# TUMFTM/CamRaDepth

Measured on AMD Instinct MI355X. Metric: training images/sec at 256x416 bf16, higher is better.
Workload: dtype bf16; 1 GPU; CamRaDepth base (image+radar) train step, 8x7x256x416 per GPU, bf16 MFMA / fp32 accumulate, diffGradNorm + OneCycleLR, Dropout2d/DropPath on; global_batch=8, parallelism=dp1, hip_graph=True

## Files before the change

camradepth_amd/csrc/wgrad3x3.hip:

```cpp
#include <stdlib.h>
#include "common.h"

namespace {

struct Wg3K {
  const bf16_t* x; int x_ld; int Cin;
  const bf16_t* dy; int dy_ld; int Cout;
  int B, H, W;
  int strips_x;
  int rows_per_wg;
  int S, nchunks;
  long long total_rows;
  long long x_bytes, dy_bytes;
  crd_sum_t* dw; crd_sum_t* dbias;
  float* dw_part;
};

constexpr int XS = 6, YS = 4;
constexpr int XPX = 40;
constexpr int XLD = 64;
typedef __attribute__((address_space(3))) void* lds_ptr;
template <int N>
__device__ __forceinline__ void wait_vm() { asm volatile("s_waitcnt vmcnt(%0)" ::"n"(N) : "memory"); }

__device__ __forceinline__ int swz128(int r) { return (r & 3) ^ ((r >> 3) & 1); }
__device__ __forceinline__ int swz256(int r) { return (r & 3) | (((r >> 3) & 1) << 2); }
__device__ __forceinline__ int swz192(int r) { return (r >> 3) & 1; }
template <int COT>
__device__ __forceinline__ int swz_y(int r) { return COT == 128 ? swz256(r) : (COT == 96 ? swz192(r) : (COT == 64 ? swz128(r) : 0)); }

__device__ __forceinline__ s16x4 tr_read3(const bf16_t* p) {
  return __builtin_amdgcn_ds_read_tr16_b64_v4i16((__attribute__((address_space(3))) s16x4*)(p));
}

template <int WCO, int WCI, int TCO, int RPS>
__global__ __launch_bounds__(512) void k_wgrad3x3(Wg3K a) {
  constexpr int XSr = XS * RPS, YSr = YS * RPS;
  static_assert(WCO * WCI == 8, "8 waves");
  constexpr int NT = 4 / WCI;
  constexpr int COT = WCO * TCO * 16;
  constexpr int YGRP = 32 * COT * 2 / 1024;
  extern __shared__ __attribute__((aligned(16))) bf16_t lds[];
  bf16_t* sX = lds;
  bf16_t* sY = lds + XSr * XPX * XLD;

  const int t = threadIdx.x, l = t & 63;
  const int wv = __builtin_amdgcn_readfirstlane(t >> 6);
  const int wco = wv / WCI, wci = wv % WCI;
  const int chunk = (int)blockIdx.x / a.S, split = (int)blockIdx.x - chunk * a.S;
  const int c0 = chunk * XLD;
  const unsigned OOB = 0x80000000u;

  f32x4 acc[9][TCO][NT];
#pragma unroll
  for (int tp = 0; tp < 9; ++tp)
#pragma unroll
    for (int i = 0; i < TCO; ++i)
#pragma unroll
      for (int j = 0; j < NT; ++j) acc[tp][i][j] = f32x4{0.f, 0.f, 0.f, 0.f};
  const int q = l >> 4, prow = (l & 15) >> 2, pcol = (l & 3) * 4;
  int yoff[TCO][2], xoff[3][NT][2];
#pragma unroll
  for (int i = 0; i < TCO; ++i)
#pragma unroll
    for (int h = 0; h < 2; ++h) {
      const int r = 8 * q + prow + 4 * h;
      yoff[i][h] = r * COT + (((wco * TCO + i) ^ swz_y<COT>(r)) << 4) + pcol;
    }
#pragma unroll
  for (int kx = 0; kx < 3; ++kx)
#pragma unroll
    for (int j = 0; j < NT; ++j)
#pragma unroll
      for (int h = 0; h < 2; ++h) {
        const int r = 8 * q + prow + kx + 4 * h;
        xoff[kx][j][h] = r * XLD + (((wci * NT + j) ^ swz128(r)) << 4) + pcol;
      }
  const bool do_bias = a.dbias != nullptr && chunk == 0 && t < a.Cout;
  float bsum = 0.f;

  long long sr = (long long)split * a.rows_per_wg;
  long long sr_end = sr + a.rows_per_wg;
  if (sr_end > a.total_rows) sr_end = a.total_rows;

  const int xpix = 8 * wv + (l >> 3);
  const int xgr = l & 7;
  const int ylin = 64 * wv + l;
  const int ypix = ylin / (COT / 8);
  const int ygr = ylin % (COT / 8);

  while (sr < sr_end) {
    const long long strip = sr / a.H;
    const int y0 = (int)(sr - strip * a.H);
    long long seg_end = (strip + 1) * a.H;
    if (seg_end > sr_end) seg_end = sr_end;
    const int y1 = y0 + (int)(seg_end - sr);
    const int b = __builtin_amdgcn_readfirstlane((int)(strip / a.strips_x));
    const int sx = (int)(strip - (long long)b * a.strips_x);
    const int x0 = sx * 32;
    const crd_rsrc_t rx = make_rsrc(a.x + (long long)b * a.H * a.W * a.x_ld, (unsigned)a.x_bytes);
    const crd_rsrc_t ry = make_rsrc(a.dy + (long long)b * a.H * a.W * a.dy_ld, (unsigned)a.dy_bytes);

    auto issue_x = [&](int h) {
#if defined(__HIP_DEVICE_COMPILE__)
      if (wv < 5) {
        const int ix = x0 - 1 + xpix, ch = c0 + ((((xgr >> 1) ^ swz128(xpix)) << 1) | (xgr & 1)) * 8;
        const bool ok = (unsigned)h < (unsigned)a.H && (unsigned)ix < (unsigned)a.W && xpix < 34 && ch < a.Cin;
        const unsigned off = ok ? (unsigned)((((long long)h * a.W + ix) * a.x_ld + ch) * 2) : OOB;
        lds_dma16(rx, (unsigned)(uintptr_t)(lds_ptr)(sX + (((h + 1) % XSr) * XPX + 8 * wv) * XLD), off);
      }
#else
      (void)h;
#endif
    };
    auto issue_y = [&](int r) {
#if defined(__HIP_DEVICE_COMPILE__)
      if (wv < YGRP) {
        const int ix = x0 + ypix, co = ((((ygr >> 1) ^ swz_y<COT>(ypix)) << 1) | (ygr & 1)) * 8;
        const bool ok = r < y1 && ix < a.W && co < a.Cout;
        const unsigned off = ok ? (unsigned)((((long long)r * a.W + ix) * a.dy_ld + co) * 2) : OOB;
        lds_dma16(ry, (unsigned)(uintptr_t)(lds_ptr)(sY + (r % YSr) * 32 * COT + 512 * wv), off);
      }
#else
      (void)r;
#endif
    };

    asm volatile("s_waitcnt vmcnt(0) lgkmcnt(0)\n\ts_barrier" ::: "memory");
    issue_x(y0 - 1);
    issue_x(y0);
#pragma unroll
    for (int s = 0; s < 3; ++s)
#pragma unroll
      for (int r = 0; r < RPS; ++r) { issue_y(y0 + s * RPS + r); issue_x(y0 + s * RPS + 1 + r); }

    for (int y = y0; y < y1; y += RPS) {
      if (wv < 5 && wv < YGRP) wait_vm<4 * RPS>();
      else if (wv < 5 || wv < YGRP) wait_vm<2 * RPS>();
      asm volatile("s_waitcnt lgkmcnt(0)\n\ts_barrier" ::: "memory");
#pragma unroll
      for (int r = 0; r < RPS; ++r) { issue_y(y + 3 * RPS + r); issue_x(y + 3 * RPS + 1 + r); }

      const bool mfma_on = c0 + wci * NT * 16 < a.Cin;
      if (!mfma_on && !do_bias) continue;
#pragma unroll
      for (int rr = 0; rr < RPS; ++rr) {
        const int yy = y + rr;
        if (rr > 0 && yy >= y1) break;
        const bf16_t* yrow = sY + (yy % YSr) * 32 * COT;
        if (mfma_on) {
        bf16x8 af[TCO];
#pragma unroll
        for (int i = 0; i < TCO; ++i) {
          s16x4 lo = tr_read3(yrow + yoff[i][0]), hi = tr_read3(yrow + yoff[i][1]);
          union { bf16x8 v; s16x4 h[2]; } u;
          u.h[0] = lo; u.h[1] = hi;
          af[i] = u.v;
        }
#pragma unroll
        for (int ky = 0; ky < 3; ++ky) {
          const bf16_t* xrow = sX + ((yy + ky) % XSr) * XPX * XLD;
#pragma unroll
          for (int kx = 0; kx < 3; ++kx) {
#pragma unroll
            for (int j = 0; j < NT; ++j) {
              s16x4 lo = tr_read3(xrow + xoff[kx][j][0]), hi = tr_read3(xrow + xoff[kx][j][1]);
              union { bf16x8 v; s16x4 h[2]; } u;
              u.h[0] = lo; u.h[1] = hi;
#pragma unroll
              for (int i = 0; i < TCO; ++i)
                acc[ky * 3 + kx][i][j] = __builtin_amdgcn_mfma_f32_16x16x32_bf16(af[i], u.v, acc[ky * 3 + kx][i][j], 0, 0, 0);
            }
          }
        }
        }
        if (do_bias) {
#pragma unroll 8
          for (int r = 0; r < 32; ++r) bsum += bf2f(yrow[r * COT + ((((t >> 4) ^ swz_y<COT>(r)) << 4) | (t & 15))]);
        }
      }
    }
    sr = seg_end;
  }

  const int Ktot = 9 * a.Cin;
#pragma unroll
  for (int tp = 0; tp < 9; ++tp)
#pragma unroll
    for (int i = 0; i < TCO; ++i)
#pragma unroll
      for (int j = 0; j < NT; ++j) {
        const int ci = c0 + (wci * NT + j) * 16 + (l & 15);
#pragma unroll
        for (int r = 0; r < 4; ++r) {
          const int co = (wco * TCO + i) * 16 + (l >> 4) * 4 + r;
          if (co < a.Cout && ci < a.Cin) {
            const long long off = (long long)co * Ktot + tp * a.Cin + ci;
            if (a.dw_part) a.dw_part[(long long)split * a.Cout * Ktot + off] = acc[tp][i][j][r];
            else grad_add(a.dw + off, acc[tp][i][j][r]);
          }
        }
      }
  if (do_bias) grad_add(a.dbias + t, bsum);
}

int plan_rows(long long total_rows, int Cin, int& rows_per_wg, int budget, int cap) {
  const int chunks = cdiv(Cin, XLD);
  const int W = budget > 0 ? budget : 256;
  long long S = W / chunks;
  if (S < 1) S = 1;
  if (cap > 0 && S > cap) S = cap;
  if (S > total_rows / 8) S = total_rows / 8 > 0 ? total_rows / 8 : 1;
  rows_per_wg = (int)((total_rows + S - 1) / S);
  return (int)((total_rows + rows_per_wg - 1) / rows_per_wg);
}

template <int WCO, int WCI, int TCO, int RPS>
int launch_w3r(const Wg3K& k0, hipStream_t st, int budget, int partial_capacity) {
  Wg3K k = k0;
  constexpr int COT = WCO * TCO * 16;
  const size_t lds = (size_t)RPS * (XS * XPX * XLD + YS * 32 * COT) * sizeof(bf16_t);
  k.nchunks = cdiv(k.Cin, XLD);
  k.S = plan_rows(k.total_rows, k.Cin, k.rows_per_wg, budget, k.dw_part ? partial_capacity : 0);
  static bool attr_done = false;
  if (!attr_done) {
    crd_reserve_lds(reinterpret_cast<const void*>(&k_wgrad3x3<WCO, WCI, TCO, RPS>), (int)lds, "k_wgrad3x3");
    attr_done = true;
  }
  hipLaunchKernelGGL((k_wgrad3x3<WCO, WCI, TCO, RPS>), dim3(k.nchunks * k.S), dim3(512), lds, st, k);
  CRD_LAUNCH_CHECK("crd_conv_wgrad(3x3 streaming)");
  return CRD_OK;
}

template <int WCO, int WCI, int TCO>
int launch_w3(const Wg3K& k, hipStream_t st, int budget, int partial_capacity) {
  static int rps = -1;
  if (rps < 0) rps = crd_dev_int("CRD_W3_RPS", 2);
  return rps == 1 ? launch_w3r<WCO, WCI, TCO, 1>(k, st, budget, partial_capacity) : launch_w3r<WCO, WCI, TCO, 2>(k, st, budget, partial_capacity);
}

}

int crd_wgrad3x3_stream(const crd_wgrad_desc* d, hipStream_t st) {
  Wg3K k;
  k.x = reinterpret_cast<const bf16_t*>(d->x) + d->x_coff; k.x_ld = d->x_ld; k.Cin = d->Cin;
  k.dy = reinterpret_cast<const bf16_t*>(d->dy) + d->dy_coff; k.dy_ld = d->dy_ld; k.Cout = d->Cout;
  k.B = d->B; k.H = d->IH; k.W = d->IW;
  k.strips_x = cdiv(d->IW, 32);
  k.total_rows = (long long)d->B * k.strips_x * d->IH;
  k.rows_per_wg = 0;
  k.x_bytes = (long long)d->IH * d->IW * d->x_ld * 2;
  k.dy_bytes = (long long)d->IH * d->IW * d->dy_ld * 2;
  CRD_UNSUPPORTED(k.x_bytes < (1ll << 31) && k.dy_bytes < (1ll << 31), "crd_conv_wgrad: image too large for 32-bit byte offsets");
  k.dw = d->dw; k.dbias = d->dbias;
  k.dw_part = d->dw_partials;
  CRD_CHECK_ARG(d->dw_partials == nullptr || d->dw_partial_capacity >= 1, "crd_conv_wgrad: dw_partials needs a capacity >= 1");
  CRD_CHECK_ARG(d->wg_budget >= 0, "crd_conv_wgrad: wg_budget must be >= 0");
  if (d->Cout <= 32) return launch_w3<2, 4, 1>(k, st, d->wg_budget, d->dw_partial_capacity);
  if (d->Cout <= 64) return launch_w3<2, 4, 2>(k, st, d->wg_budget, d->dw_partial_capacity);
  if (d->Cout <= 96) return launch_w3<2, 4, 3>(k, st, d->wg_budget, d->dw_partial_capacity);
  if (crd_dev_int("CRD_W3_T22", 0)) return launch_w3<4, 2, 2>(k, st, d->wg_budget, d->dw_partial_capacity);
  return launch_w3<2, 4, 4>(k, st, d->wg_budget, d->dw_partial_capacity);
}

int crd_wgrad3x3_splits(const crd_wgrad_desc* d) {
  int rows = 0;
  return plan_rows((long long)d->B * cdiv(d->IW, 32) * d->IH, d->Cin, rows, d->wg_budget, d->dw_partial_capacity > 0 ? d->dw_partial_capacity : 0);
}
```

camradepth_amd/engine.py:

```python
import bisect
import ctypes as C
import os

import torch

from . import lib as L
from . import trace
from .config import MID_CHANNELS, UNSUP_CLASSES, ModelConfig
from .params import short_res_block_plan

_DEV = os.environ.get("CRD_DEV_SWITCHES") == "1"


def _dev_flag(name):
    return _DEV and os.environ.get(name) is not None


def _dev_int(name, default):
    return int(os.environ.get(name, default)) if _DEV else int(default)


GROUP_WGRAD = not _dev_flag("CRD_NO_GROUP_WGRAD")
SIDE_STREAMS = _dev_flag("CRD_SIDE_STREAMS")
FUSE_GN_RED = _dev_flag("CRD_FUSE_GN_RED")
# ... 74 lines not shown
        return "k_igemm<2,2,1,1>"
    if cout <= 32:
        return "k_igemm<4,1,1,1>"
    if cout <= 64:
        return "k_igemm<2,2,2,1>"
    if cout <= 96:
        return "k_igemm<4,1,1,3>"
    if 128 < cout <= 160:
        return "k_igemm<4,1,1,5>"
    return "k_igemm<2,2,2,2>"


KCAT = _dev_int("CRD_KCAT", 1) != 0
GNB_FC1 = _dev_int("CRD_GNB_FC1", 7)
GNB_SR = _dev_int("CRD_GNB_SR", 15)
QSR_GROUP = _dev_int("CRD_QSR_GROUP", 4)
FUSE_NORM2_APPLY = not _dev_flag("CRD_NO_FUSE_NORM2_APPLY")
FUSE_BLOCK_RED = not _dev_flag("CRD_NO_FUSE_BLOCK_RED")


def fused_reduce_tile_ok(cout, ohw, B):
    small = cout > 32 and -(-ohw // 128) * -(-cout // 128) * B < 192
    return FUSE_BLOCK_RED and cout % 16 == 0 and (small or cout <= 64 or 96 < cout <= 128 or cout > 160)


def persistent_conv3(spec, B):
    if os.environ.get("CRD_CONV3P", "1") == "0":
        return False
    y = spec["y"]
    plain = (not y.f32 and spec["bias"] is None and not spec["act"] and spec["res"] is None and spec["out_mode"] == 0
             and spec.get("red") is None and spec.get("chan") is None)
    halo = spec["k"] == 3 and spec["stride"] == 1 and spec["OW"] >= 32 and spec["OH"] >= 8
    tiles = -(-spec["OW"] // 32) * -(-spec["OH"] // 16) * B
    return bool(plain and halo and tiles >= 192 and spec["cout"] >= 64 and spec["cout"] % 8 == 0)


def halo_tile(cout, OH=1 << 20, OW=1 << 20, B=1):
    tiles = -(-OW // 32) * -(-OH // 8) * B
    if cout > 32 and tiles * -(-cout // 128) < 512:
        return "k_conv3x3<4,1,2,2>" if tiles * -(-cout // 64) >= 512 else "k_conv3x3<4,1,2,1>"
    if cout <= 32:
        return "k_conv3x3<4,1,2,1>"
    if cout <= 64:
        return "k_conv3x3<4,1,2,2>"
    if cout <= 96:
        return "k_conv3x3<4,1,2,3>"
    if 128 < cout <= 160 or 256 < cout <= 320:
        return "k_conv3x3<4,1,2,4>+<4,1,2,1>" if cout - (256 if cout > 256 else 128) <= 32 else "k_conv3x3<4,1,2,4>+<4,1,2,2>"
    return "k_conv3x3<4,1,2,4>"


def wgrad_tile(cout):
    if cout <= 32:
        return "k_wgrad<1,4,2,2>"
    if cout <= 64:
        return "k_wgrad<1,4,4,2>"
    if cout <= 96:
        return "k_wgrad<2,2,3,4>"
    return "k_wgrad<2,2,4,4>"


class ConvW:

    def __init__(self, name, cout, cin_ref, k, cmap, bias, need_dgrad, scatter=False, dgrad_rows=None):
        self.name, self.cout, self.cin_ref, self.k, self.taps = name, cout, cin_ref, k, k * k
        self.cmap = cmap
        self.cin_pad = len(cmap) if cmap is not None else rup(cin_ref)
        self.cout_pad = rup(cout)
        self.bias, self.need_dgrad, self.scatter = bias, need_dgrad, scatter
        self.identity = (cmap is None and self.cin_pad == cin_ref and self.taps == 1)
        self.w_fwd = self.w_dgrad = self.w_scatter = None
        self.dw = None
        self.wg_budget = 0
        self.dw_parts, self.dw_S, self.stream3_geom = None, 0, None
        self.cmap_dev = None


class Plan:
    def __init__(self, model, B, H, W, training):
        cfg = model.cfg
        assert H % 32 == 0 and W % 32 == 0, "H and W must be multiples of 32 (SURVEY.md section 8 note on 900x1600)"
        self.model, self.cfg, self.B, self.H, self.W, self.training = model, cfg, B, H, W, training
        self.dev = model.flat.device
        self.lib = L.load()
        self.fwd, self.bwd_groups, self.bwd_tags = [], [], []
        self._tag = "enc0"
        self.zero_fwd, self.zero_bwd = [], []
        self._zf_views, self._zb_views = [], []
        self.convs = []
        self.keep = []
        self.dw_entries, self.dw_grads = [], []
        self.row_grads = []
        self.kcat_entries = []
        self.shapes = {}
        self.fwd_marks = []
        self._defer = None
        self._cur_stream = 0
        self._side_streams = None
        self.split_late = False
        self.attn_parts = None
        self.mlp_parts = None
        self.stats_scratch = None
        self.buffers = []
        self.gn_conv_on = gn_conv_default()
        self.enc_taps = {}
        self.block_ops = {}
        self.need_grad = bool(getattr(model, "_need_grad", True))
        self.frozen = frozenset(n for n in model._names if not model._param(n).requires_grad)
        self._dump = {}
        f8 = getattr(model, "fp8_scales", None)
        self.fp8_keep_bf16 = bool(training or self.need_grad)
        self.fp8 = dict(f8) if (f8 and (not self.fp8_keep_bf16 or getattr(model, "fp8_train", False))) else None
        self.fp8_convs = []
        self.fp8_kcat = []
        self.fp8_grad = bool(self.fp8 is not None and training and getattr(model, "fp8_grad", False))
        self.fp8_grad_layers, self.fp8_jit, self.fp8_margin = [], True, 2.0
        if self.fp8_grad:
            self.g8_scales = torch.ones(16, dtype=F32, device=self.dev)
            self.g8_amax = torch.zeros((16, 64), dtype=torch.int32, device=self.dev)
            self.buffers += [self.g8_scales, self.g8_amax]
        self._build()

    def new(self, shape, dtype=BF16):
        t = torch.zeros(shape, dtype=dtype, device=self.dev)
        self.buffers.append(t)
        if os.environ.get("CRD_DEBUG_NAN"):
            import traceback
            fr = [f"{f.name}:{f.lineno}" for f in traceback.extract_stack()[-5:-1]]
            self.keep.append(("buf", len(self.keep), tuple(shape), str(dtype), fr, t))
        return t

    def act(self, C_, H, W, dtype=BF16, ld=None):
        return PM(self.new((self.B, H * W, ld or C_), dtype), C_, H, W)

    def zf(self, *shape):
        v = _Lazy(shape)
        self._zf_views.append(v)
        return v

    def zb(self, *shape):
        v = _Lazy(shape)
        self._zb_views.append(v)
        return v

    def _materialise(self, views):
        n = sum(v.numel for v in views)
        arena = torch.zeros(max(n, 1), dtype=SUM, device=self.dev)
        off = 0
        for v in views:
            v.t = arena[off:off + v.numel].view(v.shape)
            off += v.numel
        return arena

    def _emit(self, lst, fn_name, args, region=None, acc_slot=None, io=None):
        op = Op(getattr(self.lib, fn_name), list(args), fn_name, region, acc_slot, stream=self._cur_stream, io=io)
        lst.append(op)
        return op

    def live(self, op):
        return op.fn is not None and (op.cond is None or getattr(self, op.cond[0]) == op.cond[1])

    @staticmethod
    def op_bytes(op):
        io = op.io
        return int(io() if callable(io) else (io or 0))

    class _Side:
        def __init__(self, plan, s):
            self.plan, self.s = plan, s

        def __enter__(self):
            self.prev, self.plan._cur_stream = self.plan._cur_stream, self.s

        def __exit__(self, *a):
            self.plan._cur_stream = self.prev

    def side(self, s):
        return Plan._Side(self, s if SIDE_STREAMS else 0)

    def join(self, lst, s):
        if SIDE_STREAMS:
            lst.append(Op(None, [], "join", stream=s))

    def _push(self, grp):
        self.bwd_groups.append(grp)
        self.bwd_tags.append(self._tag)

    def conv_desc(self, x, w_t, cout, k, stride, pad, OH, OW, y, cin=None, gather=0, out_mode=0, patch_k=0, patch_c=0,
                  bias=None, bias_bstride=0, act=0, res=None, res_scale=None, stats=None, accumulate=0, red=None, chan=None):
        return dict(x=x, w=w_t, cout=cout, k=k, stride=stride, pad=pad, OH=OH, OW=OW, y=y, cin=cin if cin is not None else x.C,
                    gather=gather, out_mode=out_mode, patch_k=patch_k, patch_c=patch_c, bias=bias, bias_bstride=bias_bstride,
                    act=act, res=res, res_scale=res_scale, stats=stats, accumulate=accumulate, red=red, chan=chan)

    def conv(self, lst, spec, region=None):
        w, x = spec["w"], spec["x"]
        if isinstance(w, tuple) and w[0] == "kcat":
            flops = spec["flops_override"]
        elif isinstance(w, tuple):
            cw = w[1]
            flops = 2.0 * self.B * x.H * x.W * cw.cout * cw.taps * min(spec["cout"] // (cw.taps if w[0] == "scatter" else 1),
                                                                         cw.cin_ref)
        else:
            flops = 2.0 * self.B * spec["OH"] * spec["OW"] * spec["cout"] * w.cin_ref * w.taps
        halo = spec["k"] == 3 and spec["stride"] == 1 and spec["out_mode"] == 0 and spec["OW"] >= 32 and spec["OH"] >= 8
        cout = spec["cout"]
        covered = cout <= 160 or 256 < cout <= 320
        if (halo and SPLIT_N and cout > 128 and 0 < cout % 128 <= 64 and not covered and spec["bias"] is None
                and spec["stats"] is None and spec["res"] is None and "w_row0" not in spec):
            c_main = cout // 128 * 128
            for c0, c1 in ((0, c_main), (c_main, cout)):
                sub = dict(spec)
                sub.update(cout=c1 - c0, y=spec["y"].sl(c0, c1), w_row0=c0, flops_override=flops * (c1 - c0) / cout)
                self.conv(lst, sub, None if region is None else region[:-2] + (region[-2] + c0, region[-2] + c1))
            return None
        flops = spec.get("flops_override", flops)
        kname = halo_tile(spec["cout"], spec["OH"], spec["OW"], self.B) if halo else igemm_tile(spec["cout"], spec["OH"] * spec["OW"], self.B)
        if self._narrow_takes(spec, False):
            kname = "k_pw_narrow"
        if halo and persistent_conv3(spec, self.B):
            c = spec["cout"]
            rest = c % 128
            kname = "k_conv3x3p<2>" if c <= 64 else "k_conv3x3p<3>" if c <= 96 else "k_conv3x3p<4>" + ("" if rest == 0 or rest > 64 else
                                                                                                 "+k_conv3x3<4,1,2,1>" if rest <= 32 else "+k_conv3x3<4,1,2,2>")
        meta = {"kernel": kname, "flops": flops,
                "shape": f"{('dgrad-kcat' if w[0] == 'kcat' else 'dgrad') if isinstance(w, tuple) else 'fwd'} Cin{spec['cin']} Cout{spec['cout']} k{spec['k']} s{spec['stride']} "
                         f"out{spec['OH']}x{spec['OW']}"}
        wbytes = spec["cout"] * spec["k"] * spec["k"] * spec["cin"] * 2

        def io(spec=spec, wbytes=wbytes):
            xs, ys = spec["x"], spec["y"]
            n = xs.t.shape[0] * xs.P * spec["cin"] * (4 if xs.f32 else 2) + wbytes
            n += nbytes(ys) * (2 if spec["accumulate"] else 1) + nbytes(spec["res"])
            if spec.get("red") is not None:
                n += nbytes(spec["red"][0])
            return n
        op = Op(self.lib.crd_conv_igemm, [spec], "crd_conv_igemm", region, ("spec", spec) if region else None, meta,
                stream=self._cur_stream, io=io)
        lst.append(op)
        return op

    def _narrow_takes(self, spec, with_gn):
        y = spec["y"]
        if not (spec["k"] == 1 and spec["stride"] == 1 and spec["out_mode"] == 0 and not spec["act"] and not spec["accumulate"]
                and (with_gn or spec["cin"] == 512)
                and int(self.lib.crd_pw_narrow_supported(spec["cin"], spec["cout"], spec["OH"] * spec["OW"])) > 0):
            return False
        if y.f32:
            return spec.get("red") is None
        red = spec.get("red")
        return spec["res"] is None and spec["stats"] is None and spec.get("chan") is None and (red is None or red[5] == 0)

    def gn_conv(self, lst, spec, stats, gmul, gname, act, xn):
        w, x = spec["w"], spec["x"]
        assert x.coff == 0 and (xn is None or xn.coff == 0)
        flops = 2.0 * self.B * spec["OH"] * spec["OW"] * spec["cout"] * w.cin_ref * w.taps
        small = spec["cout"] <= 64 or -(-spec["OH"] * spec["OW"] // 64) * -(-spec["cout"] // 128) * self.B < 256
        kname = "k_gngemm_reg" + ("<2,2,1,1>" if small else "<2,2,1,2>")
        if act and not x.f32 and self._narrow_takes(spec, True):
            kname = "k_pw_narrow<gn+gelu>"
        meta = {"kernel": kname, "flops": flops,
                "shape": f"gn+fwd Cin{spec['cin']} Cout{spec['cout']} k{spec['k']} s{spec['stride']} out{spec['OH']}x{spec['OW']}"}
        gn = dict(gn_in=True, x_f32=x.f32, gmul=gmul, stats=stats, gamma=self.p(gname + ".weight"), beta=self.p(gname + ".bias"),
                  act=act, xn=xn)
        io = nbytes(x, spec["y"], xn, spec["res"]) + spec["cout"] * spec["cin"] * 2
        op = Op(self.lib.crd_gn_conv, [spec, gn], "crd_gn_conv", None, None, meta, stream=self._cur_stream, io=io)
        lst.append(op)
        return op

    def gn_bwd_conv(self, lst, spec, gx, stats, gmul, gname, act, r, dx, mask=None):
        w, x = spec["w"], spec["x"]
        cw = w[1]
        assert isinstance(w, tuple) and x.coff == 0 and gx.coff == 0 and (dx is None or dx.coff == 0) and spec["k"] == 1
        flops = 2.0 * self.B * x.H * x.W * cw.cout * cw.taps * min(spec["cout"] // (cw.taps if w[0] == "scatter" else 1), cw.cin_ref)
        small = spec["cout"] <= 64 or -(-spec["OH"] * spec["OW"] // 64) * -(-spec["cout"] // 128) * self.B < 256 or spec["out_mode"] == 1
        kname = "k_gnbwd_gemm" + ("<1>" if small else "<2>")
        meta = {"kernel": kname, "flops": flops,
                "shape": f"gnbwd+{'scatter' if w[0] == 'scatter' else 'dgrad'} Cin{spec['cin']} Cout{spec['cout']} out{spec['OH']}x{spec['OW']}"}
        frozen = self.is_frozen(gname + ".weight", gname + ".bias")
        gnb = dict(gnb_in=True, gx=gx, gmul=gmul, act=act, stats=stats, gamma=self.p(gname + ".weight"), beta=self.p(gname + ".bias"),
                   mask=mask, r=r, dx=dx, dgamma=None if frozen else self.g(gname + ".weight"), dbeta=None if frozen else self.g(gname + ".bias"))

        def io(spec=spec, x=x, gx=gx, dx=dx):
            n = nbytes(x, gx, dx) + spec["cout"] * spec["cin"] * 2
            n += nbytes(spec["y"]) * (2 if spec["accumulate"] else 1)
            if spec.get("red") is not None:
                n += nbytes(spec["red"][0])
            return n
        op = Op(self.lib.crd_gn_bwd_conv, [spec, gnb], "crd_gn_bwd_conv", None, None, meta, stream=self._cur_stream, io=io)
        lst.append(op)
        return op

    def wgrad(self, lst, x, dy, cw, k, stride, pad, OH, OW, dbias=None, cin=None):
        if cw.frozen:
            return
        if dbias is not None:
            rows = self.zb(cw.cout)
            self.row_grads.append((dbias, cw.cout, rows, 1, cw.tag, 0, cw.cout))
            dbias = rows
        spec = dict(wg=True, x=x, dy=dy, cw=cw, k=k, stride=stride, pad=pad, OH=OH, OW=OW, dbias=dbias,
                    cin=cin if cin is not None else x.C)
        stream3 = k == 3 and stride == 1 and OW >= 32 and OH >= 8
        if stream3:
            cw.stream3_geom = (x.H, x.W, spec["cin"])
        kname = ("k_wgrad3x3<2,4,1>" if cw.cout <= 32 else "k_wgrad3x3<2,4,2>" if cw.cout <= 64 else "k_wgrad3x3<2,4,3>" if cw.cout <= 96 else "k_wgrad3x3<2,4,4>") if stream3 \
            else wgrad_tile(cw.cout)
        meta = {"kernel": kname, "flops": 2.0 * self.B * OH * OW * cw.cout * cw.cin_ref * cw.taps, "param": cw.name,
                "shape": f"wgrad Cin{spec['cin']} Cout{cw.cout} k{k} s{stride} out{OH}x{OW}"}
        meta["bytes"] = x.t.shape[0] * x.P * spec["cin"] * (4 if x.f32 else 2) + nbytes(dy) + cw.cout * cw.taps * spec["cin"] * 4
        if self._defer is not None and not stream3:
            self._defer.append((spec, meta))
            return
        stream = LATE if self._cur_stream == 0 else self._cur_stream
        lst.append(Op(self.lib.crd_conv_wgrad, [spec], "crd_conv_wgrad", meta=meta, stream=stream, io=meta["bytes"]))

    def flush_deferred(self, lst):
        items, self._defer = self._defer, None
        if not items:
            return
        meta = {"kernel": "k_wgrad_grouped", "flops": sum(m["flops"] for _, m in items), "shape": f"{len(items)} wgrads",
                "params": [m["param"] for _, m in items]}
        lst.append(Op(self.lib.crd_conv_wgrad_grouped, [{"wg_group": [sp for sp, _ in items]}], "crd_conv_wgrad_grouped", meta=meta,
                      stream=LATE, io=sum(m["bytes"] for _, m in items)))

    def _make_group(self, specs):
        descs = (L.WgradDesc * len(specs))()
        for i, sp in enumerate(specs):
            self._make_desc(sp, into=descs[i])
        info = L.WgradGroupInfo()
        L.check(self.lib.crd_wgrad_group_build(descs, len(specs), None, 0, C.byref(info)), "crd_wgrad_group_build")
        host = (C.c_uint8 * info.bytes)()
        L.check(self.lib.crd_wgrad_group_build(descs, len(specs), host, info.bytes, C.byref(info)), "crd_wgrad_group_build")
        table = torch.frombuffer(bytearray(bytes(host)), dtype=torch.uint8).to(self.dev)
        self.buffers.append(table)
        self.keep.append(info)
        return [table.data_ptr(), C.byref(info)]

    def _make_desc(self, sp, into=None):
        def P(v):
            if v is None:
                return None
            if isinstance(v, PM):
                return v.t.data_ptr()
            return v.data_ptr()
        if sp.get("gn_in"):
            n = L.GnInput()
            n.x_f32, n.gmul, n.act = sp["x_f32"], sp["gmul"], sp["act"]
            n.stats, n.gamma, n.beta = P(sp["stats"]), P(sp["gamma"]), P(sp["beta"])
            n.xn, n.xn_ld = (P(sp["xn"]), sp["xn"].ld) if sp["xn"] is not None else (None, 0)
            self.keep.append(n)
            return C.byref(n)
        if sp.get("gnb_in"):
            n = L.GnBwdInput()
            gx = sp["gx"]
            n.gx, n.gx_f32, n.gx_ld, n.gmul, n.act = P(gx), gx.f32, gx.ld, sp["gmul"], sp["act"]
            n.stats, n.gamma, n.beta, n.mask, n.r = P(sp["stats"]), P(sp["gamma"]), P(sp["beta"]), P(sp["mask"]), P(sp["r"])
            n.dx, n.dx_ld = (P(sp["dx"]), sp["dx"].ld) if sp["dx"] is not None else (None, 0)
            n.dgamma, n.dbeta = P(sp["dgamma"]), P(sp["dbeta"])
            self.keep.append(n)
            return C.byref(n)
        if sp.get("mlp"):
            d = L.MlpDesc()
            for k_, v in sp["ptrs"].items():
                setattr(d, k_, P(v))
            d.B, d.H, d.W, d.C, d.hidden = sp["dims"]
            self.keep.append(d)
            return C.byref(d)
        if sp.get("fp8d"):
            y = sp["y"]
            d = L.ConvDesc()
            d.x, d.x_ld, d.x_coff, d.B, d.IH, d.IW, d.Cin = sp["x8"].data_ptr(), sp["x8_ld"], 0, self.B, sp["H"], sp["W"], sp["cin"]
            d.w, d.Cout, d.KH, d.KW, d.stride, d.pad, d.OH, d.OW = sp["w8"].data_ptr(), sp["cout"], 3, 3, 1, 1, sp["H"], sp["W"]
            d.gather_mode, d.y, d.y_ld, d.y_coff, d.accumulate = 1, P(y), y.ld, y.coff, sp["accumulate"]
            self.keep.append(d)
            return C.byref(d)
        if sp.get("fp8"):
            cw, y = sp["cw"], sp["y"]
            d = L.ConvDesc()
            d.x, d.x_ld, d.x_coff, d.B, d.IH, d.IW, d.Cin = sp["x8"].data_ptr(), sp["x8_ld"], 0, self.B, sp["H"], sp["W"], sp["cin"]
            d.w, d.Cout, d.KH, d.KW, d.stride, d.pad, d.OH, d.OW = cw.w8.data_ptr(), cw.cout, 3, 3, 1, 1, sp["H"], sp["W"]
            d.y, d.y_ld, d.y_coff = P(y), y.ld, y.coff
            need = self.B * -(-sp["W"] // 32) * -(-sp["H"] // 16) * 4 * (cw.cout // 16) * 2
            if self.stats_scratch is None or self.stats_scratch.numel() < need:
                self.stats_scratch = self.new((need,), F32)
            d.stats, d.stats_partial, d.stats_partial_capacity = P(sp["stats"]), self.stats_scratch.data_ptr(), self.stats_scratch.numel()
            self.keep.append(d)
            return C.byref(d)
        if sp.get("wg"):
            x, dy, cw = sp["x"], sp["dy"], sp["cw"]
            d = into if into is not None else L.WgradDesc()
            d.x, d.x_ld, d.x_coff, d.B, d.IH, d.IW, d.Cin = P(x), x.ld, x.coff, self.B, x.H, x.W, sp["cin"]
            d.dy, d.dy_ld, d.dy_coff, d.OH, d.OW, d.Cout = P(dy), dy.ld, dy.coff, sp["OH"], sp["OW"], cw.cout
            d.KH, d.KW, d.stride, d.pad = sp["k"], sp["k"], sp["stride"], sp["pad"]
            d.dw, d.dbias = P(cw.dw), P(sp["dbias"])
            if cw.dw_parts is not None:
                d.dw_partials, d.dw_partial_capacity, d.wg_budget = cw.dw_parts.data_ptr(), cw.dw_S, cw.wg_budget
        else:
            x, y, w = sp["x"], sp["y"], sp["w"]
            if isinstance(w, tuple) and w[0] == "kcat":
                w = w[2]
            elif isinstance(w, tuple):
                w = w[1].w_dgrad if w[0] == "dgrad" else w[1].w_scatter
                assert w is not None, "packed data-gradient weights were not requested for this convolution"
            elif isinstance(w, ConvW):
                w = w.w_fwd
            d = L.ConvDesc()
            d.x, d.x_ld, d.x_coff, d.B, d.IH, d.IW, d.Cin = P(x), x.ld, x.coff, self.B, x.H, x.W, sp["cin"]
            d.w, d.Cout, d.KH, d.KW, d.stride, d.pad = P(w), sp["cout"], sp["k"], sp["k"], sp["stride"], sp["pad"]
            if sp.get("w_row0"):
                d.w += sp["w_row0"] * sp["k"] * sp["k"] * sp["cin"] * 2
            d.OH, d.OW, d.gather_mode = sp["OH"], sp["OW"], sp["gather"]
            d.y, d.y_ld, d.y_coff, d.y_f32 = P(y), y.ld, y.coff, y.f32
            d.out_mode, d.patch_k, d.patch_c = sp["out_mode"], sp["patch_k"], sp["patch_c"]
            d.bias, d.bias_bstride, d.act = P(sp["bias"]), sp["bias_bstride"], sp["act"]
            res = sp["res"]
            d.res, d.res_ld, d.res_scale = P(res), (res.ld if res is not None else 0), P(sp["res_scale"])
            d.accumulate, d.stats = sp["accumulate"], P(sp["stats"])
            if sp.get("stats") is not None and persistent_conv3(sp, self.B):
                need = self.B * -(-sp["OW"] // 32) * -(-sp["OH"] // 16) * 8 * (sp["cout"] // 16) * 2
                if self.stats_scratch is None or self.stats_scratch.numel() < need:
                    self.stats_scratch = self.new((need,), F32)
                d.stats_partial, d.stats_partial_capacity = self.stats_scratch.data_ptr(), self.stats_scratch.numel()
            d.chan_sums = P(sp.get("chan"))
            if sp.get("red") is not None:
                rx, rstats, rgamma, rbeta, rgmul, ract, rr = sp["red"]
                assert rx.coff == 0, "the fused reduce reads the GroupNorm input from channel 0"
                d.red_x, d.red_x_ld, d.red_gmul, d.red_act, d.red_x_f32 = P(rx), rx.ld, rgmul, ract, rx.f32
                d.red_stats, d.red_gamma, d.red_beta, d.red_r = P(rstats), P(rgamma), P(rbeta), P(rr)
        self.keep.append(d)
        return C.byref(d)

    def p(self, name):
        return self.model.param_view(name)

    def g(self, name):
        if name in self.frozen:
            if name not in self._dump:
                self._dump[name] = self.new(tuple(self.model._param(name).shape), F32)
            return self._dump[name]
        return self.model.grad_view(name)

    def is_frozen(self, *names):
        return all(n in self.frozen for n in names if self.model.has_param(n))

    def new_conv(self, name, cmap=None, need_dgrad=True, scatter=False):
        w = self.p(name + ".weight")
        cout, cin_ref = w.shape[0], w.shape[1]
        k = w.shape[2] if w.dim() == 4 else 1
        bias = self.p(name + ".bias") if self.model.has_param(name + ".bias") else None
        cw = ConvW(name, cout, cin_ref, k, cmap, bias, need_dgrad, scatter)
        cw.frozen = self.is_frozen(name + ".weight", name + ".bias")
        cw.tag = self._tag
        self.convs.append(cw)
        return cw

    def gn_fwd(self, x, stats, gmul, gname, act, mask, y):
        op = self._emit(self.fwd, "crd_gn_apply", [x.t, x.f32, x.ld, x.coff, self.B, x.P, x.C, stats, gmul,
                                                   self.p(gname + ".weight"), self.p(gname + ".bias"), act, mask, y.t, y.f32, y.ld,
                                                   y.coff], io=nbytes(x, y))
        op.meta = None
        self.shapes[id(op)] = f"P{x.P} C{x.C} xf32={x.f32}"

    def gn_stats_apply(self, x, stats, chan, gmul, gname, act, mask, y):
        self._emit(self.fwd, "crd_gn_stats", [x.t, x.f32, x.ld, x.coff, self.B, x.P, x.C, stats, chan], io=nbytes(x))
        self.gn_fwd(x, stats, gmul, gname, act, mask, y)

    def gn_bwd(self, grp, x, stats, gmul, gname, act, mask, dy, dx, region=None, dx_acc=0, r=None, dx2=None, scale2=None):
        common = [x.t, x.f32, x.ld, x.coff, dy.t, dy.f32, dy.ld, dy.coff, self.B, x.P, x.C, stats, gmul,
                  self.p(gname + ".weight"), self.p(gname + ".bias"), act, mask]
        if r is None:
            r = self.zb(self.B * x.C * 2 + self.B * (x.C // (16 * gmul)) * 2)
            self._emit(grp, "crd_gn_bwd_reduce", common + [r, None, 0], io=nbytes(x, dy))
        args = common + [r, self.g(gname + ".weight"), self.g(gname + ".bias"), dx.t, dx.f32, dx.ld, dx.coff, dx_acc]
        acc_idx = len(args) - 1
        assert dx2 is None or dx2.coff == 0
        args += [dx2.t if dx2 is not None else None, dx2.ld if dx2 is not None else 0, scale2]
        op = self._emit(grp, "crd_gn_bwd_apply", args, region, acc_idx if region else None)
        op.io = lambda op=op, i=acc_idx, x=x, dy=dy, dx=dx, dx2=dx2: nbytes(x, dy, dx, dx2) + (nbytes(dx) if op.args[i] else 0)

    def conv_layer(self, name, x, k, out, mask=None, dout=None, dx=None, dx_region=None, x8=None, out8=None, kcat=None):
        cw = self.new_conv(name + ".model.0", cmap=self._cmap, need_dgrad=dx is not None and kcat is None)
        H, W = x.H, x.W
        raw = self.act(cw.cout, H, W)
        stats = self.zf(self.B, cw.cout // 16, 2)
        if x8 is not None:
            assert k == 3 and x.coff == 0
            cin16 = rup(cw.cin_pad, 16)
            cw.w8 = self.new((cw.cout, 9, cin16), torch.uint8)
            cw.w8_scales = self.new((cw.cout,), F32)
            self.fp8_convs.append((cw, cin16))
            spec = dict(fp8=True, x8=x8[0], x8_ld=x8[1], cin=cin16, H=H, W=W, cw=cw, y=raw, stats=stats, cout=cw.cout)
            meta = {"kernel": "k_conv3x3_fp8<%d>" % (2 if cw.cout <= 64 else 3 if cw.cout <= 96 else 4),
                    "flops": 2.0 * self.B * H * W * cw.cout * cw.cin_ref * 9, "shape": f"fwd fp8 Cin{cin16} Cout{cw.cout} k3 s1 out{H}x{W}"}
            self.fwd.append(Op(self.lib.crd_conv3x3_fp8, [spec, cw.w8_scales, float(x8[2])], "crd_conv3x3_fp8", meta=meta,
                               io=self.B * H * W * cin16 + nbytes(raw) + cw.cout * 9 * cin16))
        else:
            self.conv(self.fwd, self.conv_desc(x, cw, cw.cout, k, 1, k // 2, H, W, raw, stats=stats))
        if out8 is not None:
            yb = [out.t, out.ld, out.coff] if out is not None else [None, 0, 0]
            op = self._emit(self.fwd, "crd_gn_apply_fp8", [raw.t, 0, raw.ld, raw.coff, self.B, raw.P, raw.C, stats, 1,
                                                           self.p(name + ".model.1.weight"), self.p(name + ".model.1.bias"), 1, mask,
                                                           out8[0], out8[1], out8[2], float(out8[3])] + yb)
            op.meta = None
            op.io = nbytes(raw, out) + raw.t.shape[0] * raw.P * raw.C
            self.shapes[id(op)] = f"P{raw.P} C{raw.C} -> fp8"
        else:
            self.gn_fwd(raw, stats, 1, name + ".model.1", 1, mask, out)
        if dout is None:
            return
        grp = []
        draw = kcat["draw"] if kcat is not None else self.act(cw.cout, H, W)
        f8g = kcat.get("f8") if kcat is not None else None
        if f8g is not None:
            draw8, ld8, sc_ptr, am_ptr = f8g["draw8"], f8g["ld8"], f8g["sc_ptr"], f8g["am_ptr"]
            xcat, Wt, n0, n1, dcb, real = kcat["launch"]
            K = xcat.C
            gname = name + ".model.1"
            common = [raw.t, raw.f32, raw.ld, raw.coff, dout.t, dout.f32, dout.ld, dout.coff, self.B, raw.P, raw.C, stats, 1,
                      self.p(gname + ".weight"), self.p(gname + ".bias"), 1, mask]
            r = self.zb(self.B * raw.C * 2 + self.B * (raw.C // 16) * 2)
            self._emit(grp, "crd_gn_bwd_reduce", common + [r, None, 0], io=nbytes(raw, dout))
            self._emit(grp, "crd_gn_bwd_apply_fp8", common + [r, self.g(gname + ".weight"), self.g(gname + ".bias"), draw.t, draw.ld, draw.coff,
                                                              draw8, ld8, draw.coff, sc_ptr, am_ptr], io=nbytes(raw, dout, draw) + self.B * H * W * cw.cout)
            self._emit(grp, "crd_fp8_scale_update", [am_ptr, sc_ptr, 1, self.fp8_margin, f8g["keep"]], io=256).cond = ("fp8_jit", True)
            self._emit(grp, "crd_quant_fp8_dev", [xcat.t, self.B * H * W, xcat.ld, 0, K, draw8, ld8, 0, sc_ptr],
                       io=nbytes(xcat) + self.B * H * W * K).cond = ("fp8_jit", True)
            self.wgrad(grp, x, draw, cw, k, 1, k // 2, H, W)
            for (Wt_, ld, coff, row0, rows) in kcat["packs"]:
                self.kcat_entries.append((cw, Wt_, ld, coff, row0, rows))
            W8 = self.new((n1 - n0, 9, K), torch.uint8)
            W8s = self.new((n1 - n0,), F32)
            self.fp8_kcat.append((cw, Wt, n1 - n0, K, W8, W8s))
            spec = dict(fp8d=True, x8=draw8, x8_ld=ld8, cin=K, H=H, W=W, w8=W8, y=dcb.sl(n0, n1), cout=n1 - n0, accumulate=0)
            meta = {"kernel": "k_conv3x3_fp8<dgrad>", "flops": 2.0 * self.B * H * W * 9 * real,
                    "shape": f"dgrad-kcat fp8 Cin{K} Cout{n1 - n0} k3 s1 out{H}x{W}"}
            grp.append(Op(self.lib.crd_conv3x3_fp8_dgrad, [spec, W8s, sc_ptr], "crd_conv3x3_fp8_dgrad", ("dcb", id(dcb.t), n0, n1),
                          ("spec", spec), meta, io=self.B * H * W * K + (n1 - n0) * 9 * K + nbytes(dcb.sl(n0, n1))))
            self._push(grp)
            return
        self.gn_bwd(grp, raw, stats, 1, name + ".model.1", 1, mask, dout, draw)
        self.wgrad(grp, x, draw, cw, k, 1, k // 2, H, W)
        if kcat is not None:
            for (Wt, ld, coff, row0, rows) in kcat["packs"]:
                self.kcat_entries.append((cw, Wt, ld, coff, row0, rows))
            xcat, Wt, n0, n1, dcb, real = kcat["launch"]
            spec = self.conv_desc(xcat, ("kcat", cw, Wt), n1 - n0, k, 1, k // 2, H, W, dcb.sl(n0, n1), gather=1)
            spec["flops_override"] = 2.0 * self.B * H * W * 9 * real
            self.conv(grp, spec, region=("dcb", id(dcb.t), n0, n1))
        elif dx is not None:
            self.conv(grp, self.conv_desc(draw, ("dgrad", cw), dx.C, k, 1, k // 2, H, W, dx, gather=1), region=dx_region)
        self._push(grp)

    def _build(self):
        cfg, B, H, W = self.cfg, self.B, self.H, self.W
        m = self.model
        tr = self.training
        nblk = sum(cfg.depths)
        seg = cfg.supervised_seg or cfg.unsupervised_seg
        n_drop = 5 + (2 if seg else 0)
        self.dp_masks = self.new((nblk, B), F32) if tr else None
        self.d2_masks = self.new((n_drop, B, MID_CHANNELS), F32) if tr else None
        if tr:
            self.dp_keep = torch.tensor([1.0 - r for r in cfg.drop_path_rates], dtype=F32, device=self.dev)
            self.d2_keep = torch.full((n_drop * B,), 0.8, dtype=F32, device=self.dev)
            self.rng_counter = torch.zeros(1, dtype=torch.int64, device=self.dev)
        self._drop_i = 0

        def dmask():
            i = self._drop_i
            self._drop_i += 1
            return self.d2_masks[i] if tr else None

        Cin = cfg.input_channels
        self.x_in = torch.zeros((B, Cin, H, W), dtype=F32, device=self.dev)
        X8 = self.act(8, H, W)
        self._emit(self.fwd, "crd_nchw_to_pm", [self.x_in, B, Cin, H, W, X8.t, X8.ld, 0, 8], io=nbytes(self.x_in, X8))

        enc_out_b = []
        d_enc_out = []
        src, bi = X8, 0
        for s in range(4):
            self._tag = f"enc{s}"
            self.fwd_marks.append((f"enc{s}", len(self.fwd)))
            Cs, heads, ratio, sr = cfg.dims[s], cfg.heads[s], cfg.ff_expansion[s], cfg.reduction_ratio[s]
            k, stride = (7, 4) if s == 0 else (3, 2)
            Hs, Ws = src.H // stride, src.W // stride
            N = Hs * Ws
            pe = f"dest_encoder.patch_embed{s + 1}"
            cmap = list(range(Cin)) + [-1] * (8 - Cin) if s == 0 else None
            cw = self.new_conv(pe + ".proj", cmap=cmap, need_dgrad=s > 0)
            raw = self.act(Cs, Hs, Ws)
            st = self.zf(B, Cs // 16, 2)
            self.conv(self.fwd, self.conv_desc(src, cw, Cs, k, stride, k // 2, Hs, Ws, raw, bias=cw.bias, stats=st))
            X = self.act(Cs, Hs, Ws, F32)
            self.gn_fwd(raw, st, 1, pe + ".norm", 0, None, X)
            DX = self.act(Cs, Hs, Ws, F32)
            grp = []
            draw = self.act(Cs, Hs, Ws)
            self.gn_bwd(grp, raw, st, 1, pe + ".norm", 0, None, DX, draw)
            self._defer = [] if GROUP_WGRAD else None
            self.wgrad(grp, src, draw, cw, k, stride, k // 2, Hs, Ws, dbias=pe + ".proj.bias")
            if s > 0:
                self.conv(grp, self.conv_desc(draw, ("dgrad", cw), src.C, k, stride, k // 2, src.H, src.W, d_enc_out[s - 1],
                                              gather=1), region=("dxs", s - 1, 0, src.C))
            else:
                enc0 = (grp, draw, cw)
            self._push(grp)
            hid = Cs * ratio
# ... 853 lines not shown
```

Before: 453.6 images/s.

## Split 3x3 wgrad rows across wave pairs for small Cout and fold in LDS

For Cout<=64 the streaming 3x3 weight-gradient kernel now gives each wco wave group one of the two rows in a step, with all output channels in its tile, instead of splitting output channels between groups. This halves the Y tile width held in LDS and lets each wave issue more MFMAs per X fragment it reads. At the end, the accumulators from the two groups are reduced through LDS with barriers before the store. The cost is the extra fold phase, higher accumulator register pressure (TCO doubled), and a dev switch to turn the path off.

```diff
diff --git a/camradepth_amd/csrc/wgrad3x3.hip b/camradepth_amd/csrc/wgrad3x3.hip
--- a/camradepth_amd/csrc/wgrad3x3.hip
+++ b/camradepth_amd/csrc/wgrad3x3.hip
@@ -26,6 +26,8 @@
 __device__ __forceinline__ int swz128(int r) { return (r & 3) ^ ((r >> 3) & 1); }
 __device__ __forceinline__ int swz256(int r) { return (r & 3) | (((r >> 3) & 1) << 2); }
 __device__ __forceinline__ int swz192(int r) { return (r >> 3) & 1; }
+constexpr int w3_cot(int WCO, int TCO, bool RSPLIT) { return (RSPLIT ? 1 : WCO) * TCO * 16; }
+constexpr int w3_lds_bytes(int COT, int RPS) { return RPS * (XS * XPX * XLD + YS * 32 * COT) * (int)sizeof(bf16_t); }
 template <int COT>
 __device__ __forceinline__ int swz_y(int r) { return COT == 128 ? swz256(r) : (COT == 96 ? swz192(r) : (COT == 64 ? swz128(r) : 0)); }
 
@@ -33,12 +35,14 @@
   return __builtin_amdgcn_ds_read_tr16_b64_v4i16((__attribute__((address_space(3))) s16x4*)(p));
 }
 
-template <int WCO, int WCI, int TCO, int RPS>
+template <int WCO, int WCI, int TCO, int RPS, bool RSPLIT>
 __global__ __launch_bounds__(512) void k_wgrad3x3(Wg3K a) {
   constexpr int XSr = XS * RPS, YSr = YS * RPS;
   static_assert(WCO * WCI == 8, "8 waves");
+  static_assert(!RSPLIT || (WCO == 2 && RPS == 2), "row split: one of the two rows of a step per wco wave");
   constexpr int NT = 4 / WCI;
-  constexpr int COT = WCO * TCO * 16;
+  constexpr int CO0T = RSPLIT ? 0 : TCO;
+  constexpr int COT = w3_cot(WCO, TCO, RSPLIT);
   constexpr int YGRP = 32 * COT * 2 / 1024;
   extern __shared__ __attribute__((aligned(16))) bf16_t lds[];
   bf16_t* sX = lds;
@@ -65,7 +69,7 @@
 #pragma unroll
     for (int h = 0; h < 2; ++h) {
       const int r = 8 * q + prow + 4 * h;
-      yoff[i][h] = r * COT + (((wco * TCO + i) ^ swz_y<COT>(r)) << 4) + pcol;
+      yoff[i][h] = r * COT + (((wco * CO0T + i) ^ swz_y<COT>(r)) << 4) + pcol;
     }
 #pragma unroll
   for (int kx = 0; kx < 3; ++kx)
@@ -143,12 +147,8 @@
 
       const bool mfma_on = c0 + wci * NT * 16 < a.Cin;
       if (!mfma_on && !do_bias) continue;
-#pragma unroll
-      for (int rr = 0; rr < RPS; ++rr) {
-        const int yy = y + rr;
-        if (rr > 0 && yy >= y1) break;
+      auto row_mfma = [&](int yy) {
         const bf16_t* yrow = sY + (yy % YSr) * 32 * COT;
-        if (mfma_on) {
         bf16x8 af[TCO];
 #pragma unroll
         for (int i = 0; i < TCO; ++i) {
@@ -173,17 +173,61 @@
             }
           }
         }
-        }
+      };
+      auto row_bias = [&](int yy) {
+        const bf16_t* yrow = sY + (yy % YSr) * 32 * COT;
+#pragma unroll 8
+        for (int r = 0; r < 32; ++r) bsum += bf2f(yrow[r * COT + ((((t >> 4) ^ swz_y<COT>(r)) << 4) | (t & 15))]);
+      };
+      if constexpr (RSPLIT) {
+        const int yy = y + wco;
+        if (mfma_on && yy < y1) row_mfma(yy);
         if (do_bias) {
-#pragma unroll 8
-          for (int r = 0; r < 32; ++r) bsum += bf2f(yrow[r * COT + ((((t >> 4) ^ swz_y<COT>(r)) << 4) | (t & 15))]);
+          row_bias(y);
+          if (y + 1 < y1) row_bias(y + 1);
+        }
+      } else {
+#pragma unroll
+        for (int rr = 0; rr < RPS; ++rr) {
+          const int yy = y + rr;
+          if (rr > 0 && yy >= y1) break;
+          if (mfma_on) row_mfma(yy);
+          if (do_bias) row_bias(yy);
         }
       }
     }
     sr = seg_end;
   }
 
+  if constexpr (RSPLIT) {
+    constexpr int TPS = w3_lds_bytes(COT, RPS) / (WCI * TCO * NT * 64 * 16) < 9 ? w3_lds_bytes(COT, RPS) / (WCI * TCO * NT * 64 * 16) : 9;
+    static_assert(TPS >= 1, "one tap of four waves fits the rings");
+    f32x4* fold = reinterpret_cast<f32x4*>(lds) + (wci * TPS * TCO * NT) * 64 + l;
+#pragma unroll
+    for (int tp0 = 0; tp0 < 9; tp0 += TPS) {
+      asm volatile("s_waitcnt vmcnt(0) lgkmcnt(0)\n\ts_barrier" ::: "memory");
+      if (wco == 1) {
+#pragma unroll
+        for (int tp = tp0; tp < tp0 + TPS && tp < 9; ++tp)
+#pragma unroll
+          for (int i = 0; i < TCO; ++i)
+#pragma unroll
+            for (int j = 0; j < NT; ++j) fold[(((tp - tp0) * TCO + i) * NT + j) * 64] = acc[tp][i][j];
+      }
+      asm volatile("s_waitcnt vmcnt(0) lgkmcnt(0)\n\ts_barrier" ::: "memory");
+      if (wco == 0) {
+#pragma unroll
+        for (int tp = tp0; tp < tp0 + TPS && tp < 9; ++tp)
+#pragma unroll
+          for (int i = 0; i < TCO; ++i)
+#pragma unroll
+            for (int j = 0; j < NT; ++j) acc[tp][i][j] = acc[tp][i][j] + fold[(((tp - tp0) * TCO + i) * NT + j) * 64];
+      }
+    }
+  }
+
   const int Ktot = 9 * a.Cin;
+  if (!RSPLIT || wco == 0)
 #pragma unroll
   for (int tp = 0; tp < 9; ++tp)
 #pragma unroll
@@ -193,7 +237,7 @@
         const int ci = c0 + (wci * NT + j) * 16 + (l & 15);
 #pragma unroll
         for (int r = 0; r < 4; ++r) {
-          const int co = (wco * TCO + i) * 16 + (l >> 4) * 4 + r;
+          const int co = (wco * CO0T + i) * 16 + (l >> 4) * 4 + r;
           if (co < a.Cout && ci < a.Cin) {
             const long long off = (long long)co * Ktot + tp * a.Cin + ci;
             if (a.dw_part) a.dw_part[(long long)split * a.Cout * Ktot + off] = acc[tp][i][j][r];
@@ -215,28 +259,31 @@
   return (int)((total_rows + rows_per_wg - 1) / rows_per_wg);
 }
 
-template <int WCO, int WCI, int TCO, int RPS>
+template <int WCO, int WCI, int TCO, int RPS, bool RSPLIT>
 int launch_w3r(const Wg3K& k0, hipStream_t st, int budget, int partial_capacity) {
   Wg3K k = k0;
-  constexpr int COT = WCO * TCO * 16;
-  const size_t lds = (size_t)RPS * (XS * XPX * XLD + YS * 32 * COT) * sizeof(bf16_t);
+  const size_t lds = (size_t)w3_lds_bytes(w3_cot(WCO, TCO, RSPLIT), RPS);
   k.nchunks = cdiv(k.Cin, XLD);
   k.S = plan_rows(k.total_rows, k.Cin, k.rows_per_wg, budget, k.dw_part ? partial_capacity : 0);
   static bool attr_done = false;
   if (!attr_done) {
-    crd_reserve_lds(reinterpret_cast<const void*>(&k_wgrad3x3<WCO, WCI, TCO, RPS>), (int)lds, "k_wgrad3x3");
+    crd_reserve_lds(reinterpret_cast<const void*>(&k_wgrad3x3<WCO, WCI, TCO, RPS, RSPLIT>), (int)lds, "k_wgrad3x3");
     attr_done = true;
   }
-  hipLaunchKernelGGL((k_wgrad3x3<WCO, WCI, TCO, RPS>), dim3(k.nchunks * k.S), dim3(512), lds, st, k);
+  hipLaunchKernelGGL((k_wgrad3x3<WCO, WCI, TCO, RPS, RSPLIT>), dim3(k.nchunks * k.S), dim3(512), lds, st, k);
   CRD_LAUNCH_CHECK("crd_conv_wgrad(3x3 streaming)");
   return CRD_OK;
 }
 
-template <int WCO, int WCI, int TCO>
+template <int WCO, int WCI, int TCO, int TRS = 0>
 int launch_w3(const Wg3K& k, hipStream_t st, int budget, int partial_capacity) {
-  static int rps = -1;
-  if (rps < 0) rps = crd_dev_int("CRD_W3_RPS", 2);
-  return rps == 1 ? launch_w3r<WCO, WCI, TCO, 1>(k, st, budget, partial_capacity) : launch_w3r<WCO, WCI, TCO, 2>(k, st, budget, partial_capacity);
+  static int rps = -1, rsplit = -1;
+  if (rps < 0) { rsplit = crd_dev_int("CRD_W3_ROWSPLIT", 1); rps = crd_dev_int("CRD_W3_RPS", 2); }
+  if (rps == 1) return launch_w3r<WCO, WCI, TCO, 1, false>(k, st, budget, partial_capacity);
+  if constexpr (TRS > 0) {
+    if (rsplit) return launch_w3r<2, 4, TRS, 2, true>(k, st, budget, partial_capacity);
+  }
+  return launch_w3r<WCO, WCI, TCO, 2, false>(k, st, budget, partial_capacity);
 }
 
 }
@@ -256,8 +303,8 @@
   k.dw_part = d->dw_partials;
   CRD_CHECK_ARG(d->dw_partials == nullptr || d->dw_partial_capacity >= 1, "crd_conv_wgrad: dw_partials needs a capacity >= 1");
   CRD_CHECK_ARG(d->wg_budget >= 0, "crd_conv_wgrad: wg_budget must be >= 0");
-  if (d->Cout <= 32) return launch_w3<2, 4, 1>(k, st, d->wg_budget, d->dw_partial_capacity);
-  if (d->Cout <= 64) return launch_w3<2, 4, 2>(k, st, d->wg_budget, d->dw_partial_capacity);
+  if (d->Cout <= 32) return launch_w3<2, 4, 1, 2>(k, st, d->wg_budget, d->dw_partial_capacity);
+  if (d->Cout <= 64) return launch_w3<2, 4, 2, 4>(k, st, d->wg_budget, d->dw_partial_capacity);
   if (d->Cout <= 96) return launch_w3<2, 4, 3>(k, st, d->wg_budget, d->dw_partial_capacity);
   if (crd_dev_int("CRD_W3_T22", 0)) return launch_w3<4, 2, 2>(k, st, d->wg_budget, d->dw_partial_capacity);
   return launch_w3<2, 4, 4>(k, st, d->wg_budget, d->dw_partial_capacity);
diff --git a/camradepth_amd/engine.py b/camradepth_amd/engine.py
--- a/camradepth_amd/engine.py
+++ b/camradepth_amd/engine.py
@@ -400,7 +400,7 @@
         stream3 = k == 3 and stride == 1 and OW >= 32 and OH >= 8
         if stream3:
             cw.stream3_geom = (x.H, x.W, spec["cin"])
-        kname = ("k_wgrad3x3<2,4,1>" if cw.cout <= 32 else "k_wgrad3x3<2,4,2>" if cw.cout <= 64 else "k_wgrad3x3<2,4,3>" if cw.cout <= 96 else "k_wgrad3x3<2,4,4>") if stream3 \
+        kname = ("k_wgrad3x3<2,4,2,rows>" if cw.cout <= 32 else "k_wgrad3x3<2,4,4,rows>" if cw.cout <= 64 else "k_wgrad3x3<2,4,3>" if cw.cout <= 96 else "k_wgrad3x3<2,4,4>") if stream3 \
             else wgrad_tile(cw.cout)
         meta = {"kernel": kname, "flops": 2.0 * self.B * OH * OW * cw.cout * cw.cin_ref * cw.taps, "param": cw.name,
                 "shape": f"wgrad Cin{spec['cin']} Cout{cw.cout} k{k} s{stride} out{OH}x{OW}"}
```

After: 455.9 images/s, median of 6. No clear change (+0.5%).
